# RuihanGao/visual-tactile-synthesis

Hardware: AMD Instinct MI355X
Metric: train_images_per_sec (higher is better)
Workload: dtype f32; 1 GPU; skitG G+D1+D2 train step, 1024x1024 sketch->(RGB,tactile), 4 images/GPU, 64 tactile patches/image, LPIPS/CLIP terms off (no weights offline); global_batch=4, parallelism=dp1, losses_finite=True, hip_graph=True, d2_visualisation_pass=True, train_only=False, full=False

## Files before the change

### visual-tactile-synthesis_amd/csrc/vts_conv_small.hip

```cpp
#include <stdlib.h>

#include "vts_internal.h"

namespace {

constexpr int HALO = 2;

struct SmallK {
  const float *s0, *s1, *sc0, *sh0, *sc1, *sh1;
  int64_t ns0, ns1;
  int C0, C1, Cin;
  int N, IH, IW, OH, OW, Cout, pad;
  const float* w;
  int ws_co, ws_ci;
  const float* bias;
  float* out;
  int64_t ons;
  int act_out;
  const float *dm, *dmsc, *dmsh;
  int64_t dmns;
  int dm_act, dmC;
  int accumulate;
  const float* ident;
  float slope_in;
  int IPB, PWi, plane;
  int GH, GW, PPI, MTP;
  int ablate;
  int wbytes;
  int fast;
  int inbytes;
};

template <int MODE, int S, int NR, int UMAX, int CK>
__global__ __launch_bounds__(256) void conv_small_kernel(const SmallK p) {
  constexpr int P = (MODE == 1 && S == 2) ? 4 : 1;
  constexpr int COP = (NR % 2 == 1) ? NR * 16 : NR * 16 + 16;
  extern __shared__ __attribute__((aligned(16))) float smem[];
  float* patch = smem;
  float* lds_w = smem + p.IPB * CK * p.plane;
  int* pix_tab = reinterpret_cast<int*>(lds_w + CK * 16 * COP);
  int* line_tab = pix_tab + p.MTP * 16;

  const int tid = threadIdx.x, lane = tid & 63;
  const int wave = __builtin_amdgcn_readfirstlane(tid >> 6);
  const int m16 = lane & 15, kq = lane >> 4;
  const int n0 = blockIdx.x * p.IPB;
  const int co0 = blockIdx.y * NR * 16;
  const int imgstride = CK * p.plane;
  const int npix = p.IPB * p.PPI;
  const int nunits = p.MTP * P;

  for (int i = tid; i < p.IPB * CK * p.plane; i += 256) patch[i] = 0.f;
  for (int q = tid; q < p.MTP * 16; q += 256) {
    const int img = q / p.PPI, rem = q - img * p.PPI;
    const int y = rem / p.GW, x = rem - y * p.GW;
    pix_tab[q] = q < npix ? (img << 16) | (y << 8) | x : -1;
  }
  for (int l = tid; l < p.IPB * CK * p.IH; l += 256) {
    const int img = l / (CK * p.IH), rem = l - img * (CK * p.IH);
    const int c = rem / p.IH, y = rem - c * p.IH;
    line_tab[l] = (img << 16) | (c << 8) | y;
  }
  __syncthreads();

  int abase[UMAX], uph[UMAX];
#pragma unroll
  for (int k = 0; k < UMAX; ++k) {
    const int uu = wave + 4 * k;
    const int ph = min(uu / p.MTP, P - 1), j = uu - (uu / p.MTP) * p.MTP;
    uph[k] = ph;
    const int q = 16 * j + m16;
    int off = 0;
    const int pt = uu < nunits ? pix_tab[q] : -1;
    if (pt >= 0) {
      const int img = pt >> 16, y = (pt >> 8) & 255, x = pt & 255;
      if (MODE == 0) {
        off = img * imgstride + (y * S - p.pad + HALO) * p.PWi + (x * S - p.pad + HALO) + kq;
      } else if (S == 2) {
        const int py = ph >> 1, px = ph & 1;
        off = img * imgstride + (y + ((py + p.pad) >> 1) - (kq >> 1) + HALO) * p.PWi + (x + ((px + p.pad) >> 1) - (kq & 1) + HALO);
      } else {
        off = img * imgstride + (y + p.pad + HALO) * p.PWi + (x + p.pad + HALO - kq);
      }
    }
    abase[k] = off;
  }

  f32x4 acc[UMAX][NR];
#pragma unroll
  for (int k = 0; k < UMAX; ++k)
#pragma unroll
    for (int nr = 0; nr < NR; ++nr) acc[k][nr] = (f32x4){0.f, 0.f, 0.f, 0.f};

  const int64_t iplane = (int64_t)p.IH * p.IW;
  const int nchunks = (p.Cin + CK - 1) / CK;
  const __amdgpu_buffer_rsrc_t wrs = __builtin_amdgcn_make_buffer_rsrc((void*)p.w, 0, p.wbytes, 0x00020000);
  const int half = lane >> 5, xl = lane & 31;
  const int nlines = p.IPB * CK * p.IH;
  __syncthreads();

  auto mfma_phase = [&](int cbase) {
    const int cvalid = (p.ablate & 2) ? 0 : min(CK, p.Cin - cbase);
    for (int c = 0; c < cvalid; ++c) {
      const float* pp = patch + c * p.plane;
      const float* ww = lds_w + c * 16 * COP + kq * COP + m16;
      if (MODE == 1 && S == 2) {
#pragma unroll
        for (int k = 0; k < UMAX; ++k) {
          const float a = pp[abase[k]];
#pragma unroll
          for (int nr = 0; nr < NR; ++nr)
            acc[k][nr] = __builtin_amdgcn_mfma_f32_16x16x4f32(a, ww[uph[k] * 4 * COP + nr * 16], acc[k][nr], 0, 0, 0);
        }
      } else {
#pragma unroll
        for (int g = 0; g < 4; ++g) {
          float b[NR];
#pragma unroll
          for (int nr = 0; nr < NR; ++nr) b[nr] = ww[g * 4 * COP + nr * 16];
          const int goff = (MODE == 0) ? g * p.PWi : -g * p.PWi;
#pragma unroll
          for (int k = 0; k < UMAX; ++k) {
            const float a = pp[abase[k] + goff];
#pragma unroll
            for (int nr = 0; nr < NR; ++nr) acc[k][nr] = __builtin_amdgcn_mfma_f32_16x16x4f32(a, b[nr], acc[k][nr], 0, 0, 0);
          }
        }
      }
    }
  };

  if (p.fast) {
    constexpr int NQ = 3;
    constexpr int NCO = NR * 16;
    constexpr int NWQ = CK * 4 * NCO / 256;
    float* aff_sc = reinterpret_cast<float*>(line_tab + p.IPB * CK * p.IH);
    float* aff_sh = aff_sc + p.IPB * p.Cin;
    const int HW = p.IH * p.IW, QPI = 2 * HW, nq = p.IPB * QPI;
    for (int i = tid; i < p.IPB * p.Cin; i += 256) {
      const int img = i / p.Cin, ci = i - img * p.Cin;
      const int nn = min(n0 + img, p.N - 1);
      aff_sc[i] = p.sc0 ? p.sc0[nn * p.C0 + ci] : 1.f;
      aff_sh[i] = p.sh0 ? p.sh0[nn * p.C0 + ci] : 0.f;
    }
    unsigned qoff[NQ];
    int qpk[NQ][4];
#pragma unroll
    for (int j = 0; j < NQ; ++j) {
      const int q = tid + 256 * j;
      const int img = q / QPI, r = q - img * QPI;
      const bool ok = q < nq && n0 + img < p.N;
      qoff[j] = ok ? (unsigned)(((int64_t)(n0 + img) * p.ns0 + 4 * r) * 4) : 0x40000000u;
#pragma unroll
      for (int e4 = 0; e4 < 4; ++e4) {
        const int e = 4 * r + e4;
        const int cc = e / HW, pos = e - cc * HW;
        const int y = pos / p.IW, x = pos - y * p.IW;
        qpk[j][e4] = ok ? ((img * p.Cin + cc) << 16) | (img * imgstride + cc * p.plane + (y + HALO) * p.PWi + x + HALO) : -1;
      }
    }
    const __amdgpu_buffer_rsrc_t irs = __builtin_amdgcn_make_buffer_rsrc((void*)p.s0, 0, p.inbytes, 0x00020000);
    unsigned wvo[NWQ];
    int wdst[NWQ];
#pragma unroll
    for (int e = 0; e < NWQ; ++e) {
      const int u = tid + e * 256;
      const int co = u % NCO, rest = u / NCO;
      const int ky = rest & 3, cw = rest >> 2;
      wvo[e] = co0 + co < p.Cout ? (unsigned)((co0 + co) * p.ws_co + cw * p.ws_ci + ky * 4) * 4u : 0x40000000u;
      wdst[e] = (cw * 16) * COP + co;
    }
    f32x4 qv[NQ], wq[NWQ];
    auto load_chunk = [&](int cbase) {
      if (p.ablate & 1) return;
#pragma unroll
      for (int j = 0; j < NQ; ++j) qv[j] = __builtin_bit_cast(f32x4, __builtin_amdgcn_raw_buffer_load_b128(irs, (int)qoff[j], cbase * HW * 4, 0));
#pragma unroll
      for (int e = 0; e < NWQ; ++e) wq[e] = __builtin_bit_cast(f32x4, __builtin_amdgcn_raw_buffer_load_b128(wrs, (int)wvo[e], cbase * p.ws_ci * 4, 0));
    };
    auto store_chunk = [&](int cbase) {
#pragma unroll
      for (int j = 0; j < NQ; ++j) {
        const f32x4 v = qv[j];
#pragma unroll
        for (int e4 = 0; e4 < 4; ++e4) {
          const int pk = qpk[j][e4];
          if (pk >= 0) {
            const int ai = (pk >> 16) + cbase;
            const float t = fmaf(v[e4], aff_sc[ai], aff_sh[ai]);
            patch[pk & 0xFFFF] = fmaxf(t, 0.f) + p.slope_in * fminf(t, 0.f);
          }
        }
      }
#pragma unroll
      for (int e = 0; e < NWQ; ++e) {
        const f32x4 v = wq[e];
        const int u = tid + e * 256;
        const int ky = (u / NCO) & 3;
#pragma unroll
        for (int kx = 0; kx < 4; ++kx) {
          int slot = ky * 4 + kx;
          if (MODE == 1 && S == 2) slot = ((((ky + p.pad) & 1) * 2 + ((kx + p.pad) & 1)) * 4) + (ky >> 1) * 2 + (kx >> 1);
          lds_w[wdst[e] + slot * COP] = v[kx];
        }
      }
    };
#pragma unroll
    for (int j = 0; j < NQ; ++j) qv[j] = (f32x4){0.f, 0.f, 0.f, 0.f};
#pragma unroll
    for (int e = 0; e < NWQ; ++e) wq[e] = (f32x4){0.f, 0.f, 0.f, 0.f};
    load_chunk(0);
    __syncthreads();
    store_chunk(0);
    __syncthreads();
    for (int chunk = 0; chunk < nchunks; ++chunk) {
      if (chunk + 1 < nchunks) load_chunk((chunk + 1) * CK);
      mfma_phase(chunk * CK);
      __syncthreads();
      if (chunk + 1 < nchunks) {
        store_chunk((chunk + 1) * CK);
        __syncthreads();
      }
    }
  } else
  for (int chunk = 0; chunk < nchunks; ++chunk) {
    const int cbase = chunk * CK;
    if (!(p.ablate & 1))
    for (int l0 = 0; l0 < nlines; l0 += 64) {
      float raw[8], rsc[8], rsh[8];
#pragma unroll
      for (int b = 0; b < 8; ++b) {
        const int line = min(l0 + (wave * 2 + half) + 8 * b, nlines - 1);
        const int lt = line_tab[line];
        const int img = lt >> 16, c = (lt >> 8) & 255, y = lt & 255;
        const int nn = min(n0 + img, p.N - 1), cic = min(cbase + c, p.Cin - 1);
        const bool first = cic < p.C0;
        const int cl = first ? cic : cic - p.C0;
        const float* base = first ? p.s0 + nn * p.ns0 : p.s1 + nn * p.ns1;
        raw[b] = base[cl * iplane + (int64_t)y * p.IW + min(xl, p.IW - 1)];
        const float* scp = first ? p.sc0 : p.sc1;
        const float* shp = first ? p.sh0 : p.sh1;
        const int aidx = nn * (first ? p.C0 : p.C1) + cl;
        const bool hsc = scp != nullptr, hsh = shp != nullptr;
        rsc[b] = (hsc ? scp : p.ident)[hsc ? aidx : 0];
        rsh[b] = (hsh ? shp : p.ident)[hsh ? aidx : 1];
      }
#pragma unroll
      for (int b = 0; b < 8; ++b) {
        const int line = l0 + (wave * 2 + half) + 8 * b;
        const int lt = line_tab[min(line, nlines - 1)];
        const int img = lt >> 16, c = (lt >> 8) & 255, y = lt & 255;
        const bool ok = line < nlines && n0 + img < p.N && cbase + c < p.Cin && xl < p.IW;
        const float t = fmaf(raw[b], rsc[b], rsh[b]);
        const float a = fmaxf(t, 0.f) + p.slope_in * fminf(t, 0.f);
        if (line < nlines && xl < p.IW) patch[img * imgstride + c * p.plane + (y + HALO) * p.PWi + xl + HALO] = ok ? a : 0.f;
      }
      if (p.IW > 32) {
#pragma unroll
        for (int b = 0; b < 8; ++b) {
          const int line = l0 + (wave * 2 + half) + 8 * b;
          const int lt = line_tab[min(line, nlines - 1)];
          const int img = lt >> 16, c = (lt >> 8) & 255, y = lt & 255;
          const int x = 32 + xl;
          const int nn = min(n0 + img, p.N - 1), cic = min(cbase + c, p.Cin - 1);
          const bool first = cic < p.C0;
          const int cl = first ? cic : cic - p.C0;
          const float* base = first ? p.s0 + nn * p.ns0 : p.s1 + nn * p.ns1;
          const float v = base[cl * iplane + (int64_t)y * p.IW + min(x, p.IW - 1)];
          const bool ok = line < nlines && n0 + img < p.N && cbase + c < p.Cin && x < p.IW;
          const float t = fmaf(v, rsc[b], rsh[b]);
          const float a = fmaxf(t, 0.f) + p.slope_in * fminf(t, 0.f);
          if (line < nlines && x < p.IW) patch[img * imgstride + c * p.plane + (y + HALO) * p.PWi + x + HALO] = ok ? a : 0.f;
        }
      }
    }
    {
      constexpr int NCO = NR * 16;
      constexpr int UNITS = CK * 4 * NCO;
#pragma unroll
      for (int e = 0; e < UNITS / 256; ++e) {
        const int u = tid + e * 256;
        const int co = u % NCO, rest = u / NCO;
        const int ky = rest & 3, c = rest >> 2;
        const bool ok = co0 + co < p.Cout && cbase + c < p.Cin;
        const unsigned vo = ok ? (unsigned)((co0 + co) * p.ws_co + (cbase + c) * p.ws_ci + ky * 4) * 4u : 0x40000000u;
        const f32x4 v = __builtin_bit_cast(f32x4, __builtin_amdgcn_raw_buffer_load_b128(wrs, (int)vo, 0, 0));
#pragma unroll
        for (int kx = 0; kx < 4; ++kx) {
          int slot = ky * 4 + kx;
          if (MODE == 1 && S == 2) slot = ((((ky + p.pad) & 1) * 2 + ((kx + p.pad) & 1)) * 4) + (ky >> 1) * 2 + (kx >> 1);
          lds_w[(c * 16 + slot) * COP + co] = v[kx];
        }
      }
    }
    __syncthreads();
    mfma_phase(cbase);
    __syncthreads();
  }

  const int64_t oplane = (int64_t)p.OH * p.OW;
#pragma unroll
  for (int k = 0; k < UMAX; ++k) {
    const int uu = wave + 4 * k;
    if (uu >= nunits) continue;
    const int ph = uu / p.MTP, j = uu - ph * p.MTP;
#pragma unroll
    for (int r = 0; r < 4; ++r) {
      const int q = 16 * j + kq * 4 + r;
      const int pt = pix_tab[q];
      if (pt < 0) continue;
      const int img = pt >> 16, gy = (pt >> 8) & 255, gx = pt & 255;
      const int y = (P == 4) ? gy * 2 + (ph >> 1) : gy, x = (P == 4) ? gx * 2 + (ph & 1) : gx;
      const int n = n0 + img;
      if (n >= p.N || y >= p.OH || x >= p.OW) continue;
#pragma unroll
      for (int nr = 0; nr < NR; ++nr) {
        const int co = co0 + nr * 16 + m16;
        if (co >= p.Cout) continue;
        float v = acc[k][nr][r] + (p.bias ? p.bias[co] : 0.f);
        if (p.act_out == VTS_ACT_TANH) v = tanhf(v);
        const int64_t o = co * oplane + (int64_t)y * p.OW + x;
        if (p.dm) {
          const float dsc = p.dmsc ? p.dmsc[n * p.dmC + co] : 1.f, dsh = p.dmsh ? p.dmsh[n * p.dmC + co] : 0.f;
          v *= vts_act_grad(p.dm[n * p.dmns + o] * dsc + dsh, p.dm_act);
        }
        float* ob = p.out + n * p.ons + o;
        *ob = p.accumulate ? *ob + v : v;
      }
    }
  }
}

template <int MODE, int S, int NR, int UMAX, int CK>
int launch_small(const SmallK& k, size_t lds_bytes, hipStream_t st) {
  dim3 grid(cdiv(k.N, k.IPB), cdiv(k.Cout, NR * 16));
  hipLaunchKernelGGL((conv_small_kernel<MODE, S, NR, UMAX, CK>), grid, dim3(256), lds_bytes, st, k);
  vts_set_kernel("conv_small_kernel<%d, %d, %d, %d, %d>%s", MODE, S, NR, UMAX, CK, k.fast ? "+flat" : "");
  VTS_CHECK_LAUNCH("vts_conv4x4 (small maps)");
  return VTS_OK;
}

}

int vts_conv_small_try(const vts_conv_desc* d, hipStream_t st) {
  if (d->pad_dx != 0 || d->pad < 0) return VTS_ERR_UNSUPPORTED;
  if (!d->transposed && (d->OH != (d->IH + 2 * d->pad - 4) / d->stride + 1 || d->OW != (d->IW + 2 * d->pad - 4) / d->stride + 1)) return VTS_ERR_UNSUPPORTED;
  if (d->transposed && ((d->OH + 2 * d->pad - 4) / d->stride + 1 != d->IH || (d->OW + 2 * d->pad - 4) / d->stride + 1 != d->IW)) return VTS_ERR_UNSUPPORTED;
  if (d->IH > 34 || d->IW > 34 || d->OH > 34 || d->OW > 34 || d->IW > 64 || d->N < 8) return VTS_ERR_UNSUPPORTED;
  const bool ph4 = d->transposed && d->stride == 2;
  const int P = ph4 ? 4 : 1;
  SmallK k;
  k.s0 = d->in0.data; k.sc0 = d->in0.scale; k.sh0 = d->in0.shift; k.ns0 = d->in0.nstride; k.C0 = d->in0.C;
  k.s1 = d->in1.data; k.sc1 = d->in1.scale; k.sh1 = d->in1.shift; k.ns1 = d->in1.nstride;
  k.C1 = d->in1.data ? d->in1.C : 0;
  k.Cin = k.C0 + k.C1;
  k.N = d->N; k.IH = d->IH; k.IW = d->IW; k.OH = d->OH; k.OW = d->OW; k.Cout = d->Cout; k.pad = d->pad;
  k.w = d->w; k.ws_co = d->ws_co; k.ws_ci = d->ws_ci; k.bias = d->bias;
  k.out = d->out; k.ons = d->out_nstride; k.act_out = d->act_out;
  k.dm = d->dmask.data; k.dmsc = d->dmask.scale; k.dmsh = d->dmask.shift; k.dmns = d->dmask.nstride;
  k.dm_act = d->dmask_act; k.dmC = d->dmask.C;
  k.accumulate = d->accumulate;
  k.ident = vts_ident();
  if (!k.ident) return VTS_ERR_UNSUPPORTED;
  k.slope_in = vts_slope(d->act_in);
  static const int ablate = vts_tune("VTS_ABLATE", 0);
  k.ablate = ablate;
  k.wbytes = (int)(((int64_t)(d->Cout - 1) * d->ws_co + (int64_t)(k.Cin - 1) * d->ws_ci + 16) * 4);
  k.PWi = d->IW + 2 * HALO + 1;
  k.plane = (d->IH + 2 * HALO) * k.PWi;
  k.GH = ph4 ? (d->OH + 1) / 2 : d->OH;
  k.GW = ph4 ? (d->OW + 1) / 2 : d->OW;
  k.PPI = k.GH * k.GW;
  const int nrt = (d->Cout + 15) / 16;
  const int NR = nrt >= 2 ? 2 : 1;
  constexpr int CK = 8;
  const int COP = (NR % 2 == 1) ? NR * 16 : NR * 16 + 16;
  const int groups = cdiv(d->Cout, NR * 16);
  int ipb = (4 * 8 * 16) / (k.PPI * P);
  const int lds_cap = (48 * 1024 / 4 - CK * 16 * COP) / (CK * k.plane);
  static const int small_wgs = vts_tune("VTS_SMALL_WGS", 256);
  int ipb_par = (d->N * groups) / small_wgs;
  if (ipb_par < 1) ipb_par = 1;
  if (ipb > lds_cap) ipb = lds_cap;
  if (ipb > ipb_par) ipb = ipb_par;
  if (ipb > d->N) ipb = d->N;
  if (ipb < 1) return VTS_ERR_UNSUPPORTED;
  k.IPB = ipb;
  k.MTP = cdiv(ipb * k.PPI, 16);
  const int upw = cdiv(k.MTP * P, 4);
  if (upw > 8) return VTS_ERR_UNSUPPORTED;
  const int U = upw <= 1 ? 1 : (upw <= 2 ? 2 : (upw <= 4 ? 4 : 8));
  k.inbytes = (int)((int64_t)d->N * d->in0.nstride * 4 < (int64_t)0x40000000 ? (int64_t)d->N * d->in0.nstride * 4 : 0);
  k.fast = !d->in1.data && k.Cin % CK == 0 && d->in0.nstride == (int64_t)k.Cin * d->IH * d->IW && (reinterpret_cast<uintptr_t>(d->in0.data) & 15) == 0 &&
           ipb * 2 * d->IH * d->IW <= 768 && k.inbytes > 0 && (reinterpret_cast<uintptr_t>(d->w) & 15) == 0 && ((d->ws_co | d->ws_ci) & 3) == 0;
  const size_t lds = (size_t)(ipb * CK * k.plane + CK * 16 * COP + k.MTP * 16 + ipb * CK * d->IH + (k.fast ? 2 * ipb * k.Cin : 0)) * sizeof(float);
#define SMALL_U(MODE, S, NRV)                                                  \
  switch (U) {                                                                 \
    case 1: return launch_small<MODE, S, NRV, 1, CK>(k, lds, st);              \
    case 2: return launch_small<MODE, S, NRV, 2, CK>(k, lds, st);              \
    case 4: return launch_small<MODE, S, NRV, 4, CK>(k, lds, st);              \
    default: return launch_small<MODE, S, NRV, 8, CK>(k, lds, st);             \
  }
#define SMALL_CASE(MODE, S)             \
  if (NR == 1) { SMALL_U(MODE, S, 1) }  \
  SMALL_U(MODE, S, 2)
  if (!d->transposed) {
    if (d->stride == 2) { SMALL_CASE(0, 2) }
    SMALL_CASE(0, 1)
  }
  if (d->stride == 2) { SMALL_CASE(1, 2) }
  SMALL_CASE(1, 1)
#undef SMALL_U
#undef SMALL_CASE
}
```

### visual-tactile-synthesis_amd/csrc/vts_wgrad.hip

```cpp
#include <stdio.h>
#include <stdlib.h>

#include "vts_internal.h"

namespace {

struct Src {
  const float *d0, *d1, *sc0, *sh0, *sc1, *sh1;
  int64_t ns0, ns1;
  int C0, C1, C;
  int act;
  float slope;
  const float* ident;
  int plain;
};

struct WgK {
  Src lo, hi;
  int N, LH, LW, HH, HW, pad, padx;
  int cl_groups, ch_groups;
  int tiles_y, tiles_x, ntiles;
  float* part;
  int ablate;
};
// ... 409 lines not shown
  };

  Tile cur = decode(min((int)blockIdx.x, p.ntiles - 1));
  if (!(p.ablate & 1)) load_tile(cur);
  for (int tile = blockIdx.x; tile < p.ntiles; tile += gridDim.x) {
    if (!(p.ablate & 4)) store_tile(cur);
    const int y0 = cur.y0, x0 = cur.x0;
    const int next = tile + gridDim.x;
    if (next < p.ntiles) {
      cur = decode(next);
      if (!(p.ablate & 1)) load_tile(cur);
    }
    const int nrow = (p.ablate & 2) ? 0 : min(TY, p.LH - y0), nxs = min(KSTEPS, (p.LW - x0 + 3) >> 2);
    for (int row = 0; row < nrow; ++row) {
      const float* lrow = lo + (row * CLP + m16) * TXLP + kq;
      const float* hrow = hi + (wave * CHT * PRH + row * S + (m16 >> 2)) * PCHP + kq * S + (m16 & 3);
      for (int xs = 0; xs < nxs; ++xs) {
        float a[CLT], b[CHT];
#pragma unroll
        for (int t = 0; t < CLT; ++t) a[t] = lrow[t * 16 * TXLP + xs * 4];
#pragma unroll
        for (int h = 0; h < CHT; ++h) b[h] = hrow[h * PRH * PCHP + xs * 4 * S];
#pragma unroll
        for (int t = 0; t < CLT; ++t)
#pragma unroll
          for (int h = 0; h < CHT; ++h) acc[t][h] = __builtin_amdgcn_mfma_f32_16x16x4f32(a[t], b[h], acc[t][h], 0, 0, 0);
      }
    }
    __syncthreads();
  }

  const int CL = p.lo.C, CH = p.hi.C;
  float* part = p.part + (int64_t)blockIdx.x * CL * CH * 16;
#pragma unroll
  for (int t = 0; t < CLT; ++t)
#pragma unroll
    for (int h = 0; h < CHT; ++h) {
      const int ch = ch0 + wave * CHT + h;
#pragma unroll
      for (int r = 0; r < 4; ++r) {
        const int cl = cl0 + t * 16 + kq * 4 + r;
        if (cl < CL && ch < CH) part[((int64_t)cl * CH + ch) * 16 + m16] = acc[t][h][r];
      }
    }
}

struct SmallWK {
  const float *lo, *losc, *losh, *hi, *hisc, *hish;
  int64_t lons, hins;
  int CL, CH, N, LH, LW, HH, HW, S, pad, padx;
  float lo_slope, hi_slope;
  int IPB, nblocks, POS, POSP, PW_, PLANE;
  float* part;
};
constexpr int SW_HALO = 2;

__device__ __forceinline__ int fdiv(int e, int d, float inv, int& rem) {
  int q = (int)((float)e * inv);
  int r = e - q * d;
  if (r < 0) { --q; r += d; }
  if (r >= d) { ++q; r -= d; }
  rem = r;
  return q;
}

template <int CLT, int CHW>
__global__ __launch_bounds__(256) void wgrad_small_kernel(const SmallWK p) {
  extern __shared__ __attribute__((aligned(16))) float smem[];
  float* lo_t = smem;
  float* hi_t = lo_t + CLT * 16 * p.POSP;
  int* postab = reinterpret_cast<int*>(hi_t + p.IPB * p.CH * p.PLANE);
  const int tid = threadIdx.x, lane = tid & 63;
  const int wave = __builtin_amdgcn_readfirstlane(tid >> 6);
  const int m16 = lane & 15, kq = lane >> 4;
  const int lhw = p.LH * p.LW, hhw = p.HH * p.HW;
  const int imgstride = p.CH * p.PLANE;
  const float inv_blk = 1.f / (float)(p.IPB * lhw), inv_lhw = 1.f / (float)lhw, inv_hhw = 1.f / (float)hhw, inv_ch = 1.f / (float)p.CH,
              inv_hw = 1.f / (float)p.HW;
  for (int i = tid; i < CLT * 16 * p.POSP + p.IPB * imgstride; i += 256) smem[i] = 0.f;
  for (int q = tid; q < p.POS; q += 256) {
    const int img = q / lhw, rem = q - img * lhw;
    const int y = rem / p.LW, x = rem - y * p.LW;
    postab[q] = img < p.IPB ? img * imgstride + (y * p.S - p.pad + SW_HALO) * p.PW_ + (x * p.S - p.padx + SW_HALO) : 0;
  }
  const int tapoff = (m16 >> 2) * p.PW_ + (m16 & 3);
  f32x4 acc[CLT][CHW];
#pragma unroll
  for (int t = 0; t < CLT; ++t)
#pragma unroll
    for (int c = 0; c < CHW; ++c) acc[t][c] = (f32x4){0.f, 0.f, 0.f, 0.f};
  __syncthreads();

  for (int blk = blockIdx.x; blk < p.nblocks; blk += gridDim.x) {
    const int n0 = blk * p.IPB;
    const int nimg = min(p.IPB, p.N - n0);
    const int lo_total = p.CL * p.IPB * lhw;
    for (int e0 = tid; e0 < lo_total; e0 += 256 * 8) {
      float raw[8], fsc[8], fsh[8];
      int dst[8];
      bool live[8];
#pragma unroll
      for (int j = 0; j < 8; ++j) {
        const int e = min(e0 + j * 256, lo_total - 1);
        int q, r;
        const int c = fdiv(e, p.IPB * lhw, inv_blk, q);
        const int img = fdiv(q, lhw, inv_lhw, r);
        const int n = n0 + min(img, nimg - 1);
        raw[j] = p.lo[n * p.lons + (int64_t)c * lhw + r];
        fsc[j] = p.losc ? p.losc[n * p.CL + c] : 1.f;
        fsh[j] = p.losh ? p.losh[n * p.CL + c] : 0.f;
        dst[j] = e0 + j * 256 < lo_total ? c * p.POSP + q : -1;
        live[j] = img < nimg;
      }
#pragma unroll
      for (int j = 0; j < 8; ++j) {
        const float t = fmaf(raw[j], fsc[j], fsh[j]);
        if (dst[j] >= 0) lo_t[dst[j]] = live[j] ? fmaxf(t, 0.f) + p.lo_slope * fminf(t, 0.f) : 0.f;
      }
    }
    const int hi_total = nimg * p.CH * hhw;
    for (int e0 = tid; e0 < hi_total; e0 += 256 * 8) {
      float raw[8], fsc[8], fsh[8];
      int dst[8];
#pragma unroll
      for (int j = 0; j < 8; ++j) {
        const int e = min(e0 + j * 256, hi_total - 1);
        int r, c, x;
        const int ic = fdiv(e, hhw, inv_hhw, r);
        const int img = fdiv(ic, p.CH, inv_ch, c);
        const int y = fdiv(r, p.HW, inv_hw, x);
        const int n = n0 + img;
        raw[j] = p.hi[n * p.hins + (int64_t)c * hhw + r];
        fsc[j] = p.hisc ? p.hisc[n * p.CH + c] : 1.f;
        fsh[j] = p.hish ? p.hish[n * p.CH + c] : 0.f;
        dst[j] = e0 + j * 256 < hi_total ? img * imgstride + c * p.PLANE + (y + SW_HALO) * p.PW_ + x + SW_HALO : -1;
      }
#pragma unroll
      for (int j = 0; j < 8; ++j) {
        const float t = fmaf(raw[j], fsc[j], fsh[j]);
        if (dst[j] >= 0) hi_t[dst[j]] = fmaxf(t, 0.f) + p.hi_slope * fminf(t, 0.f);
      }
    }
    __syncthreads();
    const int ngroups = (nimg * lhw + 3) >> 2;
    constexpr int UG = (CLT * CHW >= 16) ? 2 : 4;
    for (int g0 = 0; g0 < ngroups; g0 += UG) {
      float a[UG][CLT], b[UG][CHW];
#pragma unroll
      for (int u = 0; u < UG; ++u) {
        const int pos = min(g0 + u, ngroups - 1) * 4 + kq;
#pragma unroll
        for (int t = 0; t < CLT; ++t) a[u][t] = lo_t[(t * 16 + m16) * p.POSP + pos];
        const int base = postab[pos] + tapoff;
#pragma unroll
        for (int c = 0; c < CHW; ++c) b[u][c] = hi_t[base + min(wave * CHW + c, p.CH - 1) * p.PLANE];
      }
#pragma unroll
      for (int u = 0; u < UG; ++u) {
        if (g0 + u < ngroups) {
#pragma unroll
          for (int t = 0; t < CLT; ++t)
#pragma unroll
            for (int c = 0; c < CHW; ++c) acc[t][c] = __builtin_amdgcn_mfma_f32_16x16x4f32(a[u][t], b[u][c], acc[t][c], 0, 0, 0);
        }
      }
    }
    __syncthreads();
  }
  float* part = p.part + (int64_t)blockIdx.x * p.CL * p.CH * 16;
#pragma unroll
  for (int t = 0; t < CLT; ++t)
#pragma unroll
    for (int c = 0; c < CHW; ++c) {
      const int ch = wave * CHW + c;
#pragma unroll
      for (int r = 0; r < 4; ++r) {
        const int cl = t * 16 + kq * 4 + r;
        if (cl < p.CL && ch < p.CH) part[((int64_t)cl * p.CH + ch) * 16 + m16] = acc[t][c][r];
      }
    }
}

struct HeadWK {
  const float* lo;
  int64_t lons;
  const float *hi, *hisc, *hish;
  int64_t hins;
  int CH, N, LH, LW, HH, HW, pad, padx;
  float hi_slope;
  int tiles_y, tiles_x;
  float* part;
};
constexpr int HWG_TY = 16, HWG_TX = 32, HWG_PR = HWG_TY + 3, HWG_PC = HWG_TX + 3, HWG_PCP = 36, HWG_CK = 16, HWG_PLANE = HWG_PR * HWG_PCP;

__global__ __launch_bounds__(256) void wgrad_head_kernel(const HeadWK p) {
  __shared__ __attribute__((aligned(16))) float patch[HWG_CK * HWG_PLANE];
// ... 197 lines not shown
    }
    s += ((a[0] + a[1]) + (a[2] + a[3])) + ((a[4] + a[5]) + (a[6] + a[7]));
  }
  red[w][lane] = s;
  __syncthreads();
  if (w == 0) {
    f32x4 v = red[0][lane];
#pragma unroll
    for (int k = 1; k < 16; ++k) v += red[k][lane];
#pragma unroll
    for (int e = 0; e < 4; ++e) {
      const int64_t i = base + lane * 4 + e;
      if (i < j.nel) j.dw[i] = j.accumulate ? j.dw[i] + v[e] : v[e];
    }
  }
}

struct Plan {
  int clt, cht, cl_groups, ch_groups, pw, tiles_y, tiles_x, ntiles, txl;
  int ns;
  int ty;
  int head;
  int small;
  int ipb, nblocks, pos, posp, pwf, plane, lds_bytes;
};

int ns_tile_rows(int clt, int cht, int LH);

Plan make_plan(const vts_wgrad_desc* d) {
  Plan pl;
  pl.ty = 0;
  pl.head = 0;
  const int CL = d->lo0.C + (d->lo1.data ? d->lo1.C : 0), CH = d->hi0.C + (d->hi1.data ? d->hi1.C : 0);
  pl.ns = 0;
  pl.small = 0;
  if (!d->lo1.data && !d->hi1.data && d->N >= 32 && d->LH * d->LW <= 324 && d->HH <= 34 && d->HW <= 34 && CL <= 64 && CH <= 64 &&
      d->pad >= 0 && d->pad <= SW_HALO && d->pad + d->pad_dx >= 0 && d->pad + d->pad_dx <= SW_HALO) {
    const int clt = CL <= 16 ? 1 : (CL <= 32 ? 2 : 4);
    const int need = cdiv(CH, 4);
    const int chw = need <= 2 ? 2 : (need <= 4 ? 4 : (need <= 8 ? 8 : 16));
    if (clt * chw <= 32) {
      const int ph = d->HH + 2 * SW_HALO > (d->LH - 1) * d->stride - d->pad + SW_HALO + 4 ? d->HH + 2 * SW_HALO : (d->LH - 1) * d->stride - d->pad + SW_HALO + 4;
      const int padx = d->pad + d->pad_dx;
      const int pwf = d->HW + 2 * SW_HALO > (d->LW - 1) * d->stride - padx + SW_HALO + 4 ? d->HW + 2 * SW_HALO : (d->LW - 1) * d->stride - padx + SW_HALO + 4;
      const int plane = ph * pwf;
      int ipb = cdiv(d->N, 256);
      for (; ipb >= 1; --ipb) {
        const int pos = (ipb * d->LH * d->LW + 3) & ~3;
        const int posp = pos + ((4 - pos) & 31);
        const int64_t floats = (int64_t)clt * 16 * posp + (int64_t)ipb * CH * plane + pos;
        static const int lds_cap_kb = vts_tune("VTS_WGRAD_SMALL_LDS_KB", 150);
        if (floats * 4 <= (int64_t)lds_cap_kb * 1024 || (ipb == 1 && floats * 4 <= 150 * 1024)) {
          pl.small = 1; pl.clt = clt; pl.cht = chw; pl.ipb = ipb; pl.pos = pos; pl.posp = posp; pl.pwf = pwf; pl.plane = plane;
          pl.lds_bytes = (int)(floats * 4);
          pl.nblocks = cdiv(d->N, ipb);
          pl.pw = pl.nblocks < 256 ? pl.nblocks : 256;
          pl.cl_groups = pl.ch_groups = 1; pl.tiles_y = pl.tiles_x = pl.ntiles = 0; pl.txl = 0;
          return pl;
        }
      }
    }
  }
  if (CL == 1 && !d->lo1.data && !d->hi1.data && d->stride == 1 && d->act_lo == VTS_ACT_NONE && !d->lo0.scale && !d->lo0.shift &&
      d->LH >= 8 && d->LW >= 16 && d->act_hi != VTS_ACT_TANH) {
    pl.head = 1;
    pl.clt = pl.cht = pl.cl_groups = pl.ch_groups = 1;
    pl.tiles_y = cdiv(d->LH, HWG_TY);
    pl.tiles_x = cdiv(d->LW, HWG_TX);
    pl.ntiles = d->N * pl.tiles_y * pl.tiles_x;
    pl.txl = HWG_TX;
    pl.pw = pl.ntiles;
    return pl;
  }
  static const int use_ns = vts_tune("VTS_WGRAD_NS", 1);
  constexpr int ns_min_ch = 2;
  static const int ns_min_w = vts_tune("VTS_WGRAD_NS_MINW", 8);
  if (use_ns && CH >= ns_min_ch && d->LW > ns_min_w && (int64_t)d->HH * d->HW < (1 << 24) && (int64_t)d->LH * d->LW < (1 << 24)) {
    pl.ns = 1;
    pl.cl_groups = cdiv(CL, 80);
    pl.clt = cdiv(CL, 16 * pl.cl_groups);
    pl.ch_groups = cdiv(CH, 20);
    pl.cht = cdiv(CH, 4 * pl.ch_groups);
    const int ty = d->stride == 2 ? ns_tile_rows(pl.clt, pl.cht, d->LH) : 4;
    pl.ty = ty;
    pl.tiles_y = cdiv(d->LH, ty);
    pl.txl = 28;
    pl.tiles_x = cdiv(d->LW, 28);
    pl.ntiles = d->N * pl.tiles_y * pl.tiles_x;
    const int64_t nel = (int64_t)CL * CH * 16;
    static const int old_plan = vts_tune("VTS_WGRAD_OLDPLAN", 0);
    if (old_plan) {
      const int groups = pl.cl_groups * pl.ch_groups;
      int pw = 512 / groups;
      const int64_t operand = (int64_t)d->N * ((int64_t)CL * d->LH * d->LW + (int64_t)CH * d->HH * d->HW);
      int64_t cap = (2 * operand > (1 << 18) ? 2 * operand : (1 << 18)) / nel;
      if (cap > (16 << 20) / nel) cap = (16 << 20) / nel;
      if (pw > cap) pw = (int)cap;
      if (pw < 1) pw = 1;
      if (pw > pl.ntiles) pw = pl.ntiles;
      pl.pw = pw;
    } else {
      int copies = pl.ntiles / 5 > 1 ? pl.ntiles / 5 : 1;
      auto next_split = [](int C, int unit, int tiles_now, int& groups, int& tiles) {
        for (int t = tiles_now - 1; t >= 2; --t) {
          const int g = cdiv(C, unit * t), tt = cdiv(C, unit * g);
          if (tt < tiles_now && (int64_t)g * tt * unit * 100 <= (int64_t)C * 112) {
            groups = g;
// ... 96 lines not shown
bool dispatch_ns(const WgK& k, const Plan& pl, hipStream_t st) {
  if (S == 2 && pl.ty > 2) {
#define TALL_CASE(CLT, CHT, TY) \
  if (pl.clt == CLT && pl.cht == CHT && pl.ty == TY) { launch_ns_tall<CLT, CHT, TY>(k, pl, st); return true; }
    TALL_CASE(1, 1, 8) TALL_CASE(2, 1, 8)
#undef TALL_CASE
    return false;
  }
#define NS_CASE(CLT, CHT) \
  if (pl.clt == CLT && pl.cht == CHT) { launch_ns<S, CLT, CHT>(k, pl, st); return true; }
#define NS_ROW(CLT) NS_CASE(CLT, 1) NS_CASE(CLT, 2) NS_CASE(CLT, 3) NS_CASE(CLT, 4) NS_CASE(CLT, 5)
  NS_ROW(1) NS_ROW(2) NS_ROW(3) NS_ROW(4) NS_ROW(5)
#undef NS_ROW
#undef NS_CASE
  return false;
}

}


extern "C" int64_t vts_wgrad4x4_ws_floats(const vts_wgrad_desc* d) {
  if (!d) return 0;
  const int64_t CL = d->lo0.C + (d->lo1.data ? d->lo1.C : 0), CH = d->hi0.C + (d->hi1.data ? d->hi1.C : 0);
  const Plan pl = make_plan(d);
  return (int64_t)pl.pw * CL * CH * 16;
}

extern "C" int vts_wgrad4x4(const vts_wgrad_desc* d, float* ws, void* stream) {
  VTS_CHECK_ARG(d && d->lo0.data && d->hi0.data && d->dw && ws, "vts_wgrad4x4: null pointer");
  VTS_CHECK_ARG(d->stride == 1 || d->stride == 2, "vts_wgrad4x4: stride %d unsupported", d->stride);
  VTS_CHECK_ARG(d->LH <= d->HH + 16 && d->LW <= d->HW + 16 && d->pad >= -8 && d->pad <= 8,
                "vts_wgrad4x4: lo %dx%d / pad %d implausible for hi %dx%d s%d", d->LH, d->LW, d->pad, d->HH, d->HW, d->stride);
  const Plan pl = make_plan(d);
  WgK k;
  fill_src(k.lo, d->lo0, d->lo1, d->act_lo);
  fill_src(k.hi, d->hi0, d->hi1, d->act_hi);
  k.N = d->N; k.LH = d->LH; k.LW = d->LW; k.HH = d->HH; k.HW = d->HW; k.pad = d->pad; k.padx = d->pad + d->pad_dx;
  k.cl_groups = pl.cl_groups; k.ch_groups = pl.ch_groups;
  k.tiles_y = pl.tiles_y; k.tiles_x = pl.tiles_x; k.ntiles = pl.ntiles;
  k.part = ws;
  static const int ablate = vts_tune("VTS_ABLATE", 0);
  k.ablate = ablate;
  hipStream_t st = (hipStream_t)stream;
  const int64_t nel = (int64_t)k.lo.C * k.hi.C * 16;
  if (pl.small) {
    SmallWK q;
    q.lo = d->lo0.data; q.losc = d->lo0.scale; q.losh = d->lo0.shift; q.lons = d->lo0.nstride;
    q.hi = d->hi0.data; q.hisc = d->hi0.scale; q.hish = d->hi0.shift; q.hins = d->hi0.nstride;
    q.CL = k.lo.C; q.CH = k.hi.C; q.N = d->N; q.LH = d->LH; q.LW = d->LW; q.HH = d->HH; q.HW = d->HW; q.S = d->stride; q.pad = d->pad;
    q.padx = d->pad + d->pad_dx;
    q.lo_slope = vts_slope(d->act_lo); q.hi_slope = vts_slope(d->act_hi);
    q.IPB = pl.ipb; q.nblocks = pl.nblocks; q.POS = pl.pos; q.POSP = pl.posp; q.PW_ = pl.pwf; q.PLANE = pl.plane;
    q.part = ws;
    bool ok = false;
#define SW_CASE(CLT, CHW)                                                                                                      \
  if (pl.clt == CLT && pl.cht == CHW) {                                                                                        \
    static bool attr = false;                                                                                                  \
    if (!attr) {                                                                                                               \
      (void)hipFuncSetAttribute((const void*)wgrad_small_kernel<CLT, CHW>, hipFuncAttributeMaxDynamicSharedMemorySize, 160 * 1024); \
      attr = true;                                                                                                             \
    }                                                                                                                          \
    hipLaunchKernelGGL((wgrad_small_kernel<CLT, CHW>), dim3(pl.pw), dim3(256), pl.lds_bytes, st, q);                           \
    vts_set_kernel("wgrad_small_kernel<%d, %d>", CLT, CHW);                                                                    \
    ok = true;                                                                                                                 \
  }
    SW_CASE(1, 2) SW_CASE(1, 4) SW_CASE(1, 8) SW_CASE(1, 16) SW_CASE(2, 2) SW_CASE(2, 4) SW_CASE(2, 8) SW_CASE(2, 16) SW_CASE(4, 2) SW_CASE(4, 4)
    SW_CASE(4, 8)
#undef SW_CASE
    VTS_CHECK_ARG(ok, "vts_wgrad4x4: no small-map instance for clt %d chw %d", pl.clt, pl.cht);
    VTS_CHECK_LAUNCH("vts_wgrad4x4 (small maps)");
    if (d->defer) return VTS_OK;
    hipLaunchKernelGGL(wgrad_reduce_kernel, dim3((unsigned)cdiv64(nel, 64)), dim3(1024), 0, st, ws, nel, pl.pw, d->dw, d->accumulate);
    VTS_CHECK_LAUNCH("vts_wgrad4x4 reduce");
    return VTS_OK;
  }
  if (pl.head) {
    HeadWK q;
    q.lo = d->lo0.data; q.lons = d->lo0.nstride;
    q.hi = d->hi0.data; q.hisc = d->hi0.scale; q.hish = d->hi0.shift; q.hins = d->hi0.nstride;
    q.CH = k.hi.C; q.N = d->N; q.LH = d->LH; q.LW = d->LW; q.HH = d->HH; q.HW = d->HW; q.pad = d->pad; q.padx = d->pad + d->pad_dx;
    q.hi_slope = vts_slope(d->act_hi);
    q.tiles_y = pl.tiles_y; q.tiles_x = pl.tiles_x;
    q.part = ws;
    hipLaunchKernelGGL(wgrad_head_kernel, dim3(pl.ntiles), dim3(256), 0, st, q);
    vts_set_kernel("wgrad_head_kernel");
    VTS_CHECK_LAUNCH("vts_wgrad4x4 (single channel)");
    if (d->defer) return VTS_OK;
    hipLaunchKernelGGL(wgrad_reduce_kernel, dim3((unsigned)cdiv64(nel, 64)), dim3(1024), 0, st, ws, nel, pl.pw, d->dw, d->accumulate);
    VTS_CHECK_LAUNCH("vts_wgrad4x4 reduce");
    return VTS_OK;
  }
  if (pl.ns) {
    const bool ok = d->stride == 2 ? dispatch_ns<2>(k, pl, st) : dispatch_ns<1>(k, pl, st);
    VTS_CHECK_ARG(ok, "vts_wgrad4x4: no N-split instance for clt %d cht %d", pl.clt, pl.cht);
    VTS_CHECK_LAUNCH("vts_wgrad4x4 (N-split)");
    if (d->defer) return VTS_OK;
    hipLaunchKernelGGL(wgrad_reduce_kernel, dim3((unsigned)cdiv64(nel, 64)), dim3(1024), 0, st, ws, nel, pl.pw, d->dw, d->accumulate);
    VTS_CHECK_LAUNCH("vts_wgrad4x4 reduce");
    return VTS_OK;
  }
#define WG_CASE(S, CLT, CHT) \
  if (d->stride == S && pl.clt == CLT && pl.cht == CHT) launch_wg<S, CLT, CHT>(k, pl, st);
  WG_CASE(2, 1, 4) WG_CASE(2, 1, 10) WG_CASE(2, 2, 4) WG_CASE(2, 2, 10) WG_CASE(2, 3, 4) WG_CASE(2, 3, 10) WG_CASE(2, 5, 4)
  WG_CASE(1, 1, 4) WG_CASE(1, 1, 10) WG_CASE(1, 2, 4) WG_CASE(1, 2, 10) WG_CASE(1, 3, 4) WG_CASE(1, 3, 10) WG_CASE(1, 5, 4)
#undef WG_CASE
  VTS_CHECK_LAUNCH("vts_wgrad4x4");
  if (d->defer) return VTS_OK;
  hipLaunchKernelGGL(wgrad_reduce_kernel, dim3((unsigned)cdiv64(nel, 64)), dim3(1024), 0, st, ws, nel, pl.pw, d->dw,
                     d->accumulate);
  VTS_CHECK_LAUNCH("vts_wgrad4x4 reduce");
  return VTS_OK;
}

extern "C" int vts_wgrad_reduce_batch(const vts_reduce_job* jobs, int njobs, void* stream) {
  VTS_CHECK_ARG(jobs && njobs >= 0, "vts_wgrad_reduce_batch: null pointer");
  hipStream_t st = (hipStream_t)stream;
// ... 23 lines not shown
```

Before: 760.7 images/s.

## Widen flat vector-load path in small conv and add quad-load pipeline to wgrad

The small-map conv kernel now templates the number of 16-byte buffer-load queues per thread (3, 6 or 10). This lets the fast flat-load path cover larger inputs, and it drops the 16-byte alignment requirement on the input and weight pointers. Per-image affine scale/shift values are staged into LDS for both the fast and slow paths, replacing per-element global loads, and one barrier is removed. The small-map weight-gradient kernel gains a QUADS variant that loads activations as double-buffered 128-bit buffer loads and prefetches the next block's first round before the current compute ends. This raises LDS use and the number of template instances.

```diff
diff --git a/visual-tactile-synthesis_amd/csrc/vts_conv_small.hip b/visual-tactile-synthesis_amd/csrc/vts_conv_small.hip
--- a/visual-tactile-synthesis_amd/csrc/vts_conv_small.hip
+++ b/visual-tactile-synthesis_amd/csrc/vts_conv_small.hip
@@ -31,7 +31,7 @@
   int inbytes;
 };
 
-template <int MODE, int S, int NR, int UMAX, int CK>
+template <int MODE, int S, int NR, int UMAX, int CK, int NQ>
 __global__ __launch_bounds__(256) void conv_small_kernel(const SmallK p) {
   constexpr int P = (MODE == 1 && S == 2) ? 4 : 1;
   constexpr int COP = (NR % 2 == 1) ? NR * 16 : NR * 16 + 16;
@@ -50,6 +50,22 @@
   const int npix = p.IPB * p.PPI;
   const int nunits = p.MTP * P;
 
+  float* aff_sc = reinterpret_cast<float*>(line_tab + p.IPB * CK * p.IH);
+  float* aff_sh = aff_sc + p.IPB * p.Cin;
+  const int naff = p.IPB * p.Cin;
+  auto affine_of = [&](int i, float& sc, float& sh) {
+    const int img = i / p.Cin, ci = i - img * p.Cin;
+    const int nn = min(n0 + img, p.N - 1);
+    const bool first = ci < p.C0;
+    const float* scp = first ? p.sc0 : p.sc1;
+    const float* shp = first ? p.sh0 : p.sh1;
+    const int aidx = first ? nn * p.C0 + ci : nn * p.C1 + ci - p.C0;
+    sc = scp ? scp[aidx] : 1.f;
+    sh = shp ? shp[aidx] : 0.f;
+  };
+  float asc[2], ash[2];
+#pragma unroll
+  for (int j = 0; j < 2; ++j) affine_of(min(tid + 256 * j, naff - 1), asc[j], ash[j]);
   for (int i = tid; i < p.IPB * CK * p.plane; i += 256) patch[i] = 0.f;
   for (int q = tid; q < p.MTP * 16; q += 256) {
     const int img = q / p.PPI, rem = q - img * p.PPI;
@@ -61,6 +77,10 @@
     const int c = rem / p.IH, y = rem - c * p.IH;
     line_tab[l] = (img << 16) | (c << 8) | y;
   }
+#pragma unroll
+  for (int j = 0; j < 2; ++j)
+    if (tid + 256 * j < naff) { aff_sc[tid + 256 * j] = asc[j]; aff_sh[tid + 256 * j] = ash[j]; }
+  for (int i = tid + 512; i < naff; i += 256) affine_of(i, aff_sc[i], aff_sh[i]);
   __syncthreads();
 
   int abase[UMAX], uph[UMAX];
@@ -130,19 +150,10 @@
     }
   };
 
-  if (p.fast) {
-    constexpr int NQ = 3;
+  if constexpr (NQ > 0) {
     constexpr int NCO = NR * 16;
     constexpr int NWQ = CK * 4 * NCO / 256;
-    float* aff_sc = reinterpret_cast<float*>(line_tab + p.IPB * CK * p.IH);
-    float* aff_sh = aff_sc + p.IPB * p.Cin;
     const int HW = p.IH * p.IW, QPI = 2 * HW, nq = p.IPB * QPI;
-    for (int i = tid; i < p.IPB * p.Cin; i += 256) {
-      const int img = i / p.Cin, ci = i - img * p.Cin;
-      const int nn = min(n0 + img, p.N - 1);
-      aff_sc[i] = p.sc0 ? p.sc0[nn * p.C0 + ci] : 1.f;
-      aff_sh[i] = p.sh0 ? p.sh0[nn * p.C0 + ci] : 0.f;
-    }
     unsigned qoff[NQ];
     int qpk[NQ][4];
 #pragma unroll
@@ -210,7 +221,6 @@
 #pragma unroll
     for (int e = 0; e < NWQ; ++e) wq[e] = (f32x4){0.f, 0.f, 0.f, 0.f};
     load_chunk(0);
-    __syncthreads();
     store_chunk(0);
     __syncthreads();
     for (int chunk = 0; chunk < nchunks; ++chunk) {
@@ -238,12 +248,8 @@
         const int cl = first ? cic : cic - p.C0;
         const float* base = first ? p.s0 + nn * p.ns0 : p.s1 + nn * p.ns1;
         raw[b] = base[cl * iplane + (int64_t)y * p.IW + min(xl, p.IW - 1)];
-        const float* scp = first ? p.sc0 : p.sc1;
-        const float* shp = first ? p.sh0 : p.sh1;
-        const int aidx = nn * (first ? p.C0 : p.C1) + cl;
-        const bool hsc = scp != nullptr, hsh = shp != nullptr;
-        rsc[b] = (hsc ? scp : p.ident)[hsc ? aidx : 0];
-        rsh[b] = (hsh ? shp : p.ident)[hsh ? aidx : 1];
+        rsc[b] = aff_sc[img * p.Cin + cic];
+        rsh[b] = aff_sh[img * p.Cin + cic];
       }
 #pragma unroll
       for (int b = 0; b < 8; ++b) {
@@ -331,13 +337,23 @@
   }
 }
 
+template <int MODE, int S, int NR, int UMAX, int CK, int NQ>
+int launch_small_nq(const SmallK& k, size_t lds_bytes, hipStream_t st) {
+  dim3 grid(cdiv(k.N, k.IPB), cdiv(k.Cout, NR * 16));
+  hipLaunchKernelGGL((conv_small_kernel<MODE, S, NR, UMAX, CK, NQ>), grid, dim3(256), lds_bytes, st, k);
+  vts_set_kernel("conv_small_kernel<%d, %d, %d, %d, %d>%s", MODE, S, NR, UMAX, CK, NQ ? "+flat" : "");
+  VTS_CHECK_LAUNCH("vts_conv4x4 (small maps)");
+  return VTS_OK;
+}
+
 template <int MODE, int S, int NR, int UMAX, int CK>
 int launch_small(const SmallK& k, size_t lds_bytes, hipStream_t st) {
-  dim3 grid(cdiv(k.N, k.IPB), cdiv(k.Cout, NR * 16));
-  hipLaunchKernelGGL((conv_small_kernel<MODE, S, NR, UMAX, CK>), grid, dim3(256), lds_bytes, st, k);
-  vts_set_kernel("conv_small_kernel<%d, %d, %d, %d, %d>%s", MODE, S, NR, UMAX, CK, k.fast ? "+flat" : "");
-  VTS_CHECK_LAUNCH("vts_conv4x4 (small maps)");
-  return VTS_OK;
+  switch (k.fast) {
+    case 0: return launch_small_nq<MODE, S, NR, UMAX, CK, 0>(k, lds_bytes, st);
+    case 3: return launch_small_nq<MODE, S, NR, UMAX, CK, 3>(k, lds_bytes, st);
+    case 6: return launch_small_nq<MODE, S, NR, UMAX, CK, 6>(k, lds_bytes, st);
+    default: return launch_small_nq<MODE, S, NR, UMAX, CK, 10>(k, lds_bytes, st);
+  }
 }
 
 }
@@ -391,9 +407,11 @@
   if (upw > 8) return VTS_ERR_UNSUPPORTED;
   const int U = upw <= 1 ? 1 : (upw <= 2 ? 2 : (upw <= 4 ? 4 : 8));
   k.inbytes = (int)((int64_t)d->N * d->in0.nstride * 4 < (int64_t)0x40000000 ? (int64_t)d->N * d->in0.nstride * 4 : 0);
-  k.fast = !d->in1.data && k.Cin % CK == 0 && d->in0.nstride == (int64_t)k.Cin * d->IH * d->IW && (reinterpret_cast<uintptr_t>(d->in0.data) & 15) == 0 &&
-           ipb * 2 * d->IH * d->IW <= 768 && k.inbytes > 0 && (reinterpret_cast<uintptr_t>(d->w) & 15) == 0 && ((d->ws_co | d->ws_ci) & 3) == 0;
-  const size_t lds = (size_t)(ipb * CK * k.plane + CK * 16 * COP + k.MTP * 16 + ipb * CK * d->IH + (k.fast ? 2 * ipb * k.Cin : 0)) * sizeof(float);
+  const int nqt = cdiv(ipb * 2 * d->IH * d->IW, 256);
+  const bool flat = !d->in1.data && k.Cin % CK == 0 && d->in0.nstride == (int64_t)k.Cin * d->IH * d->IW && nqt <= 10 && k.inbytes > 0 &&
+                    ((d->ws_co | d->ws_ci) & 3) == 0 && ipb * CK * k.plane <= 0x10000 && ipb * k.Cin < 0x8000;
+  k.fast = !flat ? 0 : (nqt <= 3 ? 3 : (nqt <= 6 ? 6 : 10));
+  const size_t lds = (size_t)(ipb * CK * k.plane + CK * 16 * COP + k.MTP * 16 + ipb * CK * d->IH + 2 * ipb * k.Cin) * sizeof(float);
 #define SMALL_U(MODE, S, NRV)                                                  \
   switch (U) {                                                                 \
     case 1: return launch_small<MODE, S, NRV, 1, CK>(k, lds, st);              \
diff --git a/visual-tactile-synthesis_amd/csrc/vts_wgrad.hip b/visual-tactile-synthesis_amd/csrc/vts_wgrad.hip
--- a/visual-tactile-synthesis_amd/csrc/vts_wgrad.hip
+++ b/visual-tactile-synthesis_amd/csrc/vts_wgrad.hip
@@ -485,8 +485,11 @@
   float lo_slope, hi_slope;
   int IPB, nblocks, POS, POSP, PW_, PLANE;
   float* part;
+  int quads;
+  int lobytes, hibytes;
 };
 constexpr int SW_HALO = 2;
+constexpr int SW_RQ = 8;
 
 __device__ __forceinline__ int fdiv(int e, int d, float inv, int& rem) {
   int q = (int)((float)e * inv);
@@ -497,7 +500,7 @@
   return q;
 }
 
-template <int CLT, int CHW>
+template <int CLT, int CHW, bool QUADS>
 __global__ __launch_bounds__(256) void wgrad_small_kernel(const SmallWK p) {
   extern __shared__ __attribute__((aligned(16))) float smem[];
   float* lo_t = smem;
@@ -510,23 +513,122 @@
   const int imgstride = p.CH * p.PLANE;
   const float inv_blk = 1.f / (float)(p.IPB * lhw), inv_lhw = 1.f / (float)lhw, inv_hhw = 1.f / (float)hhw, inv_ch = 1.f / (float)p.CH,
               inv_hw = 1.f / (float)p.HW;
+  const int tapoff = (m16 >> 2) * p.PW_ + (m16 & 3);
+  f32x4 acc[CLT][CHW];
+#pragma unroll
+  for (int t = 0; t < CLT; ++t)
+#pragma unroll
+    for (int c = 0; c < CHW; ++c) acc[t][c] = (f32x4){0.f, 0.f, 0.f, 0.f};
+
+  float* aff = reinterpret_cast<float*>(postab + p.POS);
+  const int naff_lo = p.IPB * p.CL, naff_hi = p.IPB * p.CH;
+  f32x4 qa[SW_RQ], qb[SW_RQ];
+  auto issue = [&](f32x4 (&v)[SW_RQ], int blk, int r, int rl) {
+    const int nimg = min(p.IPB, p.N - blk * p.IPB);
+    const bool is_lo = r < rl;
+    const int run = is_lo ? nimg * p.CL * lhw : nimg * p.CH * hhw;
+    const int q0 = (is_lo ? r : r - rl) * (256 * SW_RQ) + tid;
+    const int base = (int)((int64_t)blk * p.IPB * (is_lo ? p.lons : p.hins) * 4);
+    const __amdgpu_buffer_rsrc_t rs = __builtin_amdgcn_make_buffer_rsrc((void*)(is_lo ? p.lo : p.hi), 0, is_lo ? p.lobytes : p.hibytes, 0x00020000);
+#pragma unroll
+    for (int j = 0; j < SW_RQ; ++j) {
+      const int q = q0 + 256 * j;
+      const int vo = 4 * q < run ? base + 16 * q : 0x40000000;
+      v[j] = __builtin_bit_cast(f32x4, __builtin_amdgcn_raw_buffer_load_b128(rs, vo, 0, 0));
+    }
+  };
+  auto finish = [&](const f32x4 (&v)[SW_RQ], int blk, int r, int rl) {
+    const int nimg = min(p.IPB, p.N - blk * p.IPB);
+    if (r < rl) {
+      const int run = nimg * p.CL * lhw, clhw = p.CL * lhw;
+      const float inv_clhw = 1.f / (float)clhw;
+#pragma unroll
+      for (int j = 0; j < SW_RQ; ++j) {
+        const int e = 4 * (r * (256 * SW_RQ) + tid + 256 * j);
+        if (e >= run) continue;
+        int rem, x;
+        int img = fdiv(e, clhw, inv_clhw, rem);
+        int c = fdiv(rem, lhw, inv_lhw, x);
+#pragma unroll
+        for (int k = 0; k < 4; ++k) {
+          if (e + k < run) {
+            const int ai = img * p.CL + c;
+            const float t = fmaf(v[j][k], aff[ai], aff[naff_lo + ai]);
+            lo_t[c * p.POSP + img * lhw + x] = fmaxf(t, 0.f) + p.lo_slope * fminf(t, 0.f);
+          }
+          if (++x == lhw) { x = 0; if (++c == p.CL) { c = 0; ++img; } }
+        }
+      }
+    } else {
+      const int run = nimg * p.CH * hhw, chhw = p.CH * hhw;
+      const float inv_chhw = 1.f / (float)chhw;
+      const float* hsc = aff + 2 * naff_lo;
+#pragma unroll
+      for (int j = 0; j < SW_RQ; ++j) {
+        const int e = 4 * ((r - rl) * (256 * SW_RQ) + tid + 256 * j);
+        if (e >= run) continue;
+        int rem, pos, x;
+        int img = fdiv(e, chhw, inv_chhw, rem);
+        int c = fdiv(rem, hhw, inv_hhw, pos);
+        int y = fdiv(pos, p.HW, inv_hw, x);
+#pragma unroll
+        for (int k = 0; k < 4; ++k) {
+          if (e + k < run) {
+            const int ai = img * p.CH + c;
+            const float t = fmaf(v[j][k], hsc[ai], hsc[naff_hi + ai]);
+            hi_t[img * imgstride + c * p.PLANE + (y + SW_HALO) * p.PW_ + x + SW_HALO] = fmaxf(t, 0.f) + p.hi_slope * fminf(t, 0.f);
+          }
+          if (++x == p.HW) { x = 0; if (++y == p.HH) { y = 0; if (++c == p.CH) { c = 0; ++img; } } }
+        }
+      }
+    }
+  };
+  auto rounds_lo = [&](int blk) { return (min(p.IPB, p.N - blk * p.IPB) * p.CL * lhw + 1024 * SW_RQ - 1) / (1024 * SW_RQ); };
+  auto rounds_hi = [&](int blk) { return (min(p.IPB, p.N - blk * p.IPB) * p.CH * hhw + 1024 * SW_RQ - 1) / (1024 * SW_RQ); };
+  if (QUADS && (int)blockIdx.x < p.nblocks) issue(qa, blockIdx.x, 0, rounds_lo(blockIdx.x));
   for (int i = tid; i < CLT * 16 * p.POSP + p.IPB * imgstride; i += 256) smem[i] = 0.f;
   for (int q = tid; q < p.POS; q += 256) {
     const int img = q / lhw, rem = q - img * lhw;
     const int y = rem / p.LW, x = rem - y * p.LW;
     postab[q] = img < p.IPB ? img * imgstride + (y * p.S - p.pad + SW_HALO) * p.PW_ + (x * p.S - p.padx + SW_HALO) : 0;
   }
-  const int tapoff = (m16 >> 2) * p.PW_ + (m16 & 3);
-  f32x4 acc[CLT][CHW];
-#pragma unroll
-  for (int t = 0; t < CLT; ++t)
-#pragma unroll
-    for (int c = 0; c < CHW; ++c) acc[t][c] = (f32x4){0.f, 0.f, 0.f, 0.f};
   __syncthreads();
 
   for (int blk = blockIdx.x; blk < p.nblocks; blk += gridDim.x) {
     const int n0 = blk * p.IPB;
     const int nimg = min(p.IPB, p.N - n0);
+    if constexpr (QUADS) {
+      for (int i = tid; i < naff_lo; i += 256) {
+        const int img = i / p.CL, c = i - img * p.CL;
+        const int n = n0 + min(img, nimg - 1);
+        aff[i] = p.losc ? p.losc[n * p.CL + c] : 1.f;
+        aff[naff_lo + i] = p.losh ? p.losh[n * p.CL + c] : 0.f;
+      }
+      for (int i = tid; i < naff_hi; i += 256) {
+        const int img = i / p.CH, c = i - img * p.CH;
+        const int n = n0 + min(img, nimg - 1);
+        aff[2 * naff_lo + i] = p.hisc ? p.hisc[n * p.CH + c] : 1.f;
+        aff[2 * naff_lo + naff_hi + i] = p.hish ? p.hish[n * p.CH + c] : 0.f;
+      }
+      if (nimg < p.IPB)
+        for (int i = tid; i < CLT * 16 * 4; i += 256) {
+          const int pos = nimg * lhw + (i & 3);
+          if (pos < p.POS) lo_t[(i >> 2) * p.POSP + pos] = 0.f;
+        }
+      __syncthreads();
+      const int rl = rounds_lo(blk), nr = rl + rounds_hi(blk);
+      for (int r = 0; r < nr; r += 2) {
+        if (r + 1 < nr) issue(qb, blk, r + 1, rl);
+        finish(qa, blk, r, rl);
+        if (r + 1 < nr) {
+          if (r + 2 < nr) issue(qa, blk, r + 2, rl);
+          finish(qb, blk, r + 1, rl);
+        }
+      }
+      __syncthreads();
+      const int nb = blk + gridDim.x;
+      if (nb < p.nblocks) issue(qa, nb, 0, rounds_lo(nb));
+    } else {
     const int lo_total = p.CL * p.IPB * lhw;
     for (int e0 = tid; e0 < lo_total; e0 += 256 * 8) {
       float raw[8], fsc[8], fsh[8];
@@ -575,6 +677,7 @@
       }
     }
     __syncthreads();
+    }
     const int ngroups = (nimg * lhw + 3) >> 2;
     constexpr int UG = (CLT * CHW >= 16) ? 2 : 4;
     for (int g0 = 0; g0 < ngroups; g0 += UG) {
@@ -878,7 +981,7 @@
         static const int lds_cap_kb = vts_tune("VTS_WGRAD_SMALL_LDS_KB", 150);
         if (floats * 4 <= (int64_t)lds_cap_kb * 1024 || (ipb == 1 && floats * 4 <= 150 * 1024)) {
           pl.small = 1; pl.clt = clt; pl.cht = chw; pl.ipb = ipb; pl.pos = pos; pl.posp = posp; pl.pwf = pwf; pl.plane = plane;
-          pl.lds_bytes = (int)(floats * 4);
+          pl.lds_bytes = (int)((floats + 2 * ipb * (CL + CH)) * 4);
           pl.nblocks = cdiv(d->N, ipb);
           pl.pw = pl.nblocks < 256 ? pl.nblocks : 256;
           pl.cl_groups = pl.ch_groups = 1; pl.tiles_y = pl.tiles_x = pl.ntiles = 0; pl.txl = 0;
@@ -1081,16 +1184,21 @@
     q.lo_slope = vts_slope(d->act_lo); q.hi_slope = vts_slope(d->act_hi);
     q.IPB = pl.ipb; q.nblocks = pl.nblocks; q.POS = pl.pos; q.POSP = pl.posp; q.PW_ = pl.pwf; q.PLANE = pl.plane;
     q.part = ws;
+    const int64_t lob = (int64_t)d->N * d->lo0.nstride * 4, hib = (int64_t)d->N * d->hi0.nstride * 4;
+    q.quads = d->lo0.nstride == (int64_t)q.CL * d->LH * d->LW && d->hi0.nstride == (int64_t)q.CH * d->HH * d->HW && lob < 0x40000000 && hib < 0x40000000;
+    q.lobytes = q.quads ? (int)lob : 0; q.hibytes = q.quads ? (int)hib : 0;
     bool ok = false;
 #define SW_CASE(CLT, CHW)                                                                                                      \
   if (pl.clt == CLT && pl.cht == CHW) {                                                                                        \
-    static bool attr = false;                                                                                                  \
-    if (!attr) {                                                                                                               \
-      (void)hipFuncSetAttribute((const void*)wgrad_small_kernel<CLT, CHW>, hipFuncAttributeMaxDynamicSharedMemorySize, 160 * 1024); \
-      attr = true;                                                                                                             \
+    const void* fn = q.quads ? (const void*)wgrad_small_kernel<CLT, CHW, true> : (const void*)wgrad_small_kernel<CLT, CHW, false>; \
+    static bool attr[2] = {false, false};                                                                                      \
+    if (!attr[q.quads]) {                                                                                                      \
+      (void)hipFuncSetAttribute(fn, hipFuncAttributeMaxDynamicSharedMemorySize, 160 * 1024);                                   \
+      attr[q.quads] = true;                                                                                                    \
     }                                                                                                                          \
-    hipLaunchKernelGGL((wgrad_small_kernel<CLT, CHW>), dim3(pl.pw), dim3(256), pl.lds_bytes, st, q);                           \
-    vts_set_kernel("wgrad_small_kernel<%d, %d>", CLT, CHW);                                                                    \
+    if (q.quads) hipLaunchKernelGGL((wgrad_small_kernel<CLT, CHW, true>), dim3(pl.pw), dim3(256), pl.lds_bytes, st, q);        \
+    else hipLaunchKernelGGL((wgrad_small_kernel<CLT, CHW, false>), dim3(pl.pw), dim3(256), pl.lds_bytes, st, q);               \
+    vts_set_kernel("wgrad_small_kernel<%d, %d>%s", CLT, CHW, q.quads ? "+quad" : "");                                          \
     ok = true;                                                                                                                 \
   }
     SW_CASE(1, 2) SW_CASE(1, 4) SW_CASE(1, 8) SW_CASE(1, 16) SW_CASE(2, 2) SW_CASE(2, 4) SW_CASE(2, 8) SW_CASE(2, 16) SW_CASE(4, 2) SW_CASE(4, 4)
```

Result: faster. 783.3 images/s (median of 6 runs) (+3.0%).
